# EleutherAI/DALLE-mtf

Measured on AMD Instinct MI355X. Metric: train tokens/sec (text+image) per node, dalle_example, higher is better.
Workload: dtype bf16

## Files before the change

### dalle-mtf_amd/csrc/elementwise.hip

```cpp
#include "common.h"
#include <stdarg.h>

static thread_local char g_err[512] = "ok";
void dmi_set_error(const char* fmt, ...) {
  va_list ap;
  va_start(ap, fmt);
  vsnprintf(g_err, sizeof(g_err), fmt, ap);
  va_end(ap);
}
extern "C" const char* dmi_last_error_string(void) { return g_err; }
extern "C" int dmi_version(void) { return 100; }

__global__ __launch_bounds__(256) void embed_fwd_kernel(const int* __restrict__ tokens,
                                                        const bf16_t* __restrict__ wte,
                                                        const bf16_t* __restrict__ wpe, bf16_t* __restrict__ x,
                                                        int64_t rows, int S, int d, int vocab, const int* __restrict__ pos_dev) {
  const int lane = threadIdx.x & 63, wid = threadIdx.x >> 6;
  const int64_t row = (int64_t)blockIdx.x * 4 + wid;
  if (row >= rows) return;
  int tok = tokens[row];
  tok = tok < 0 ? 0 : (tok >= vocab ? vocab - 1 : tok);
  int s = (int)(row % S);
  if (pos_dev) {
    s = *pos_dev;
    s = s < 0 ? 0 : (s >= S ? S - 1 : s);
  }
  const u32x4* a = (const u32x4*)(wte + (int64_t)tok * d);
  const u32x4* p = (const u32x4*)(wpe + (int64_t)s * d);
  u32x4* o = (u32x4*)(x + row * d);
  for (int c = lane; c < d / 8; c += 64) {
    float fa[8], fp[8];
    unpack8(a[c], fa);
    unpack8(p[c], fp);
#pragma unroll
    for (int j = 0; j < 8; ++j) fa[j] += fp[j];
    o[c] = pack8(fa);
  }
}

extern "C" int dmi_embed_fwd(const int32_t* tokens, const uint16_t* wte, const uint16_t* wpe, uint16_t* x,
                             int64_t rows, int S, int d, int vocab, const int* pos_dev, void* stream) {
  DMI_REQUIRE(tokens && wte && wpe && x, "embed_fwd: null pointer");
  DMI_REQUIRE(d % 8 == 0 && rows > 0 && S > 0, "embed_fwd: d %% 8 != 0 or empty (d=%d rows=%lld)", d, (long long)rows);
  embed_fwd_kernel<<<dim3((unsigned)cdiv64(rows, 4)), dim3(256), 0, (hipStream_t)stream>>>(tokens, wte, wpe, x, rows, S, d, vocab, pos_dev);
  DMI_CHECK_LAUNCH("embed_fwd");
  return DMI_OK;
}

__global__ __launch_bounds__(256) void embed_bwd_wpe_kernel(const bf16_t* __restrict__ dx, float* __restrict__ dwpe,
                                                            int B, int S, int d) {
  const int lane = threadIdx.x & 63, wid = threadIdx.x >> 6;
  const int s = blockIdx.x * 4 + wid;
  if (s >= S) return;
  for (int c = lane; c < d / 8; c += 64) {
    float acc[8] = {0, 0, 0, 0, 0, 0, 0, 0};
    for (int b = 0; b < B; ++b) {
      float f[8];
      unpack8(*(const u32x4*)(dx + ((int64_t)b * S + s) * d + c * 8), f);
#pragma unroll
      for (int j = 0; j < 8; ++j) acc[j] += f[j];
    }
    float* o = dwpe + (int64_t)s * d + c * 8;
    *(f32x4*)o = f32x4{acc[0], acc[1], acc[2], acc[3]};
    *(f32x4*)(o + 4) = f32x4{acc[4], acc[5], acc[6], acc[7]};
  }
}
#define SORT_T 2048
#define SORT_BLK 256
__device__ __forceinline__ int sort_clamp(int k, int vocab) { return k < 0 ? 0 : (k >= vocab ? vocab - 1 : k); }
__global__ __launch_bounds__(SORT_BLK) void sort_count_kernel(const int* __restrict__ keys, int* __restrict__ hist, int n, int vocab,
                                                              int shift, int cpt) {
  __shared__ int col[16][SORT_BLK];
  const int t = threadIdx.x, g = blockIdx.x * SORT_BLK + t;
#pragma unroll
  for (int d = 0; d < 16; ++d) col[d][t] = 0;
  const int i0 = (int64_t)g * cpt < n ? g * cpt : n;
  const int i1 = i0 + cpt < n ? i0 + cpt : n;
  for (int i = i0; i < i1; ++i) col[(sort_clamp(keys[i], vocab) >> shift) & 15][t] += 1;
// ... 1127 lines not shown
      pv[j] -= lr * upd;
    }
    ((f32x4*)p)[i] = pv;
    ((f32x4*)m)[i] = mv;
    ((f32x4*)v)[i] = vv;
    if (pb) *(u32x2*)(pb + i * 4) = u32x2{pack2bf(pv[0], pv[1]), pack2bf(pv[2], pv[3])};
  }
  if (blockIdx.x == 0 && threadIdx.x < (n & 3)) {
    const int64_t i = n4 * 4 + threadIdx.x;
    const float gg = g[i] * mult;
    const float mm = b1 * m[i] + (1.f - b1) * gg;
    const float vv = b2 * v[i] + (1.f - b2) * gg * gg;
    float pp = p[i];
    pp -= lr * (mm / (sqrtf(vv) + eps) + wd * pp);
    p[i] = pp;
    m[i] = mm;
    v[i] = vv;
    if (pb) pb[i] = f2bf(pp);
  }
}
extern "C" int dmi_adam_step(float* p, const float* g, float* m, float* v, uint16_t* p_bf16, int64_t n,
                             const float* gnorm_sq, float clip, float lr, float beta1, float beta2, float eps,
                             float weight_decay, float grad_scale, const float* lr_dev, void* stream) {
  DMI_REQUIRE(p && g && m && v && n > 0, "adam_step: bad args");
  DMI_REQUIRE((((uintptr_t)p | (uintptr_t)g | (uintptr_t)m | (uintptr_t)v) & 15) == 0 && (((uintptr_t)p_bf16) & 7) == 0,
              "adam_step: buffers must be 16-byte aligned");
  int64_t blocks = cdiv64(n / 4 + 1, 256);
  if (blocks > 4096) blocks = 4096;
  adam_kernel<<<dim3((unsigned)blocks), dim3(256), 0, (hipStream_t)stream>>>(p, g, m, v, p_bf16, n, gnorm_sq, clip, lr, beta1, beta2, eps, weight_decay, grad_scale, lr_dev);
  DMI_CHECK_LAUNCH("adam_step");
  return DMI_OK;
}

__global__ __launch_bounds__(256) void cast_kernel(const float* __restrict__ in, bf16_t* __restrict__ out, int64_t n) {
  for (int64_t i = (int64_t)blockIdx.x * 256 + threadIdx.x; i < n; i += (int64_t)gridDim.x * 256) out[i] = f2bf(in[i]);
}
extern "C" int dmi_cast_f32_bf16(const float* in, uint16_t* out, int64_t n, void* stream) {
  DMI_REQUIRE(in && out && n > 0, "cast: bad args");
  int64_t blocks = cdiv64(n, 256);
  if (blocks > 8192) blocks = 8192;
  cast_kernel<<<dim3((unsigned)blocks), dim3(256), 0, (hipStream_t)stream>>>(in, out, n);
  DMI_CHECK_LAUNCH("cast");
  return DMI_OK;
}

__device__ __forceinline__ unsigned order_key(float v) {
  const unsigned u = __float_as_uint(v);
  return (u & 0x80000000u) ? ~u : (u | 0x80000000u);
}
__device__ __forceinline__ float key_value(unsigned k) { return __uint_as_float((k & 0x80000000u) ? (k & 0x7fffffffu) : ~k); }
__device__ __forceinline__ uint64_t splitmix64(uint64_t x) {
  x += 0x9E3779B97F4A7C15ull;
  x = (x ^ (x >> 30)) * 0xBF58476D1CE4E5B9ull;
  x = (x ^ (x >> 27)) * 0x94D049BB133111EBull;
  return x ^ (x >> 31);
}
#define SAMPLE_MAX_VOCAB 8192
__global__ __launch_bounds__(256) void sample_tokens_kernel(const bf16_t* __restrict__ z, int ldz, const bf16_t* __restrict__ bias, int nv,
                                                            float inv_temp, int top_k, uint64_t seed, const unsigned* __restrict__ params_dev,
                                                            int pos_arg, int* pos_dev, int advance, int token_offset,
                                                            int* __restrict__ next_tok, int* __restrict__ out, int out_ld, int out_col0) {
  __shared__ unsigned keys[SAMPLE_MAX_VOCAB];
  __shared__ int cnt[4];
  __shared__ float bval[4];
  __shared__ int bidx[4];
  const int b = blockIdx.x, tid = threadIdx.x, lane = tid & 63, wid = tid >> 6;
// ... 285 lines not shown
```

### dalle-mtf_amd/dalle_hip/__init__.py

```python
from __future__ import annotations

import ctypes
import os
import re
import struct

import numpy as np
from ctypes import c_char_p, c_float, c_int, c_int64, c_void_p

import torch

_HERE = os.path.dirname(os.path.abspath(__file__))
LIB_PATH = os.environ.get("DALLE_HIP_LIB") or os.path.join(_HERE, "libdalle_hip.so")
HEADER_PATH = os.path.join(os.path.dirname(os.path.dirname(_HERE)), "include", "dalle_hip.h")

GEMM_BIAS, GEMM_RELU, GEMM_RESIDUAL, GEMM_RELU_MASK, GEMM_OUT_F32, GEMM_ROWSCALE = 1, 2, 4, 8, 16, 32

_lib = None


class DalleHipError(RuntimeError):
    pass


# ... 31 lines not shown
        "dmi_sort_tokens": (I, [P, P, P, L64, I, P, P]),
        "dmi_embed_bwd_workspace_bytes": (L64, [I, I, I]),
        "dmi_embed_bwd": (I, [P, P, P, P, P, I, I, I, I, P, P]),
        "dmi_layernorm_fwd": (I, [P, P, P, P, P, P, L64, I, F, P]),
        "dmi_layernorm_bwd_workspace_bytes": (L64, [L64, I]),
        "dmi_layernorm_bwd": (I, [P, P, P, P, P, P, P, P, P, P, L64, I, P]),
        "dmi_layernorm_bwd_finish_batch": (I, [P, P, P, P, I, I, P]),
        "dmi_gemm_nt": (I, [P, I, P, I, P, I, I, I, I, I, P, P, P, P, P]),
        "dmi_gemm_nt_splitk_workspace_bytes": (L64, [I, I, I]),
        "dmi_gemm_nt_splitk": (I, [P, I, P, I, P, I, I, I, I, P, P, P]),
        "dmi_gemm_tn_workspace_bytes": (L64, [I, I, I]),
        "dmi_gemm_tn": (I, [P, I, P, I, P, P, P, I, I, I, P, P, P, P]),
        "dmi_gemm_tn_group": (I, [P, I, I, P, P, P]),
        "dmi_gemm_tn_group_plan": (I, [P, P, I, I]),
        "dmi_reduce_slabs_batch": (I, [P, I, P]),
        "dmi_colsum_workspace_bytes": (L64, [L64, I]),
        "dmi_colsum": (I, [P, I, P, L64, I, P, P]),
        "dmi_transpose_bf16": (I, [P, P, I, I, I, P]),
        "dmi_attention_fwd": (I, [P, P, P, I, I, I, P]),
        "dmi_attention_bwd": (I, [P, P, P, P, P, P, I, I, I, P]),
        "dmi_attention_decode": (I, [P, P, P, I, I, I, I, P, P]),
        "dmi_attention_fwd_hd": (I, [P, P, P, I, I, I, I, P]),
        "dmi_attention_bwd_hd": (I, [P, P, P, P, P, P, I, I, I, I, P]),
        "dmi_attention_decode_hd": (I, [P, P, P, I, I, I, I, P, I, P]),
        "dmi_attn_mask_plan": (L64, [P, I, P, L64]),
        "dmi_attention_fwd_masked": (I, [P, P, P, P, P, I, I, I, I, P]),
        "dmi_attention_bwd_masked": (I, [P, P, P, P, P, P, P, P, I, I, I, I, P]),
        "dmi_attention_decode_masked": (I, [P, P, P, P, P, I, I, I, I, P, I, P]),
        "dmi_label_logit": (I, [P, I, P, I, P, P, P, P, L64, I, I, P]),
        "dmi_gemm_nt_softmax_partials": (L64, [I]),
        "dmi_gemm_nt_softmax": (I, [P, I, P, I, P, P, P, I, P, I, I, I, P]),
        "dmi_softmax_finish": (I, [P, I, P, P, P, P, I, P, I, P, P, I, I, P, P, P, P, P, L64, I, I, F, P]),
        "dmi_shift_labels": (I, [P, P, I, I, I, P]),
        "dmi_cross_entropy": (I, [P, I, P, P, P, L64, I, F, P]),
        "dmi_sum_f32": (I, [P, L64, F, P, P]),
        "dmi_assemble_tokens": (I, [P, P, P, I, I, I, I, I, P]),
        "dmi_sample_tokens": (I, [P, I, P, I, I, F, I, ctypes.c_uint64, P, I, P, I, I, P, P, I, I, P]),
        "dmi_sample_tokens_p": (I, [P, I, P, I, I, F, I, ctypes.c_uint64, F, P, I, P, I, I, P, P, I, I, P, P]),
        "dmi_ln_gemm_nt": (I, [P, I, P, P, F, P, I, P, I, I, I, I, I, P, P]),
        "dmi_logits_f32": (I, [P, I, P, P, I, I, P]),
        "dmi_gemm_nt_ln": (I, [P, I, P, I, P, I, I, I, I, P, P, P, P, F, P, I, P, P, P]),
        "dmi_gemm_nt_lnbwd_parts": (I, [I]),
        "dmi_gemm_nt_lnbwd": (I, [P, I, P, I, I, I, I, P, P, P, P, P, P, P, P, I, P, P]),
        "dmi_layernorm_bwd_finish_parts": (I, [P, I, P, P, I, P]),
        "dmi_relu_bits_bytes": (L64, [I, I]),
        "dmi_relu_bits_auto": (I, [I, I, I]),
        "dmi_gemm_nt_ln_auto": (I, [I, I, I]),
        "dmi_gemm_nt_relu_bits": (I, [P, I, P, I, P, I, I, I, I, P, P, P]),
        "dmi_gemm_nt_mask_bits": (I, [P, I, P, I, P, I, I, I, I, P, P]),
        "dmi_sumsq_workspace_bytes": (L64, [L64]),
        "dmi_sumsq": (I, [P, L64, P, P, P]),
        "dmi_adam_step": (I, [P, P, P, P, P, L64, P, F, F, F, F, F, F, F, P, P]),
        "dmi_adafactor_plan": (I, [P, I, P]),
        "dmi_adafactor_step": (I, [P, I, P, P, P, P, P, P, P, F, F, P, F, F, F, F, P, L64, P]),
        "dmi_cast_f32_bf16": (I, [P, P, L64, P]),
        "dmi_transpose_bf16_padded": (I, [P, P, I, I, I, P]),
        "dmi_transpose_bf16_batch": (I, [P, P, P, I, L64, P]),
        "dmi_im2col": (I, [P, P, I, I, I, I, I, I, I, I, P, P, I, P]),
        "dmi_conv_gemm_nt": (I, [P, I, I, I, I, I, I, I, I, P, P, P, I, P, I, I, I, P, P, P, P]),
        "dmi_conv_wgrad_tn_workspace_bytes": (L64, [I, I, I]),
        "dmi_conv_wgrad_tn": (I, [P, I, I, I, I, I, I, I, I, P, P, P, I, I, P, P, P, P, P, P]),
        "dmi_weight_gather": (I, [P, P, I, I, I, P, I, P]),
        "dmi_weight_gather_batch": (I, [P, P, P, I, L64, P]),
        "dmi_pixel_interleave": (I, [P, P, I, I, I, I, P]),
        "dmi_pad_channels": (I, [P, P, L64, I, I, P]),
        "dmi_unpad_channels": (I, [P, P, L64, I, I, P]),
        "dmi_gumbel_softmax_fwd": (I, [P, P, P, P, P, L64, I, F, I, P, P]),
        "dmi_gumbel_softmax_bwd": (I, [P, P, P, L64, I, F, P, P]),
        "dmi_mse_workspace_bytes": (L64, []),
        "dmi_mse_loss": (I, [P, P, P, P, L64, I, I, F, P, P]),
        "dmi_add_f32": (I, [P, P, L64, P]),
        "dmi_comm_load": (I, [c_char_p]),
        "dmi_comm_unique_id_bytes": (I, []),
        "dmi_comm_unique_id": (I, [P]),
        "dmi_comm_init": (I, [P, I, I, P]),
        "dmi_comm_destroy": (I, [P]),
        "dmi_allreduce_bucket": (I, [P, P, L64, P]),
        "dmi_comm_broadcast_f32": (I, [P, P, L64, I, P]),
        "dmi_conv2d_f32": (I, [P, I, I, I, I, I, I, I, I, P, P, P, P, P, P, I, I, P]),
        "dmi_space_to_depth_f32": (I, [P, P, I, I, I, I, I, I, P]),
        "dmi_depth_to_space_f32": (I, [P, P, I, I, I, I, I, I, P]),
        "dmi_crc32c": (ctypes.c_uint32, [c_char_p, ctypes.c_size_t]),
    }
    for name, (res, args) in sig.items():
        fn = getattr(L, name)
# ... 281 lines not shown
        return float(self.host[PLAN_HDR["LIVE_F"]]) / float(self.host[PLAN_HDR["CAUSAL_F"]])

    def live_fraction_dkv(self):
        return float(self.host[PLAN_HDR["LIVE_K"]]) / float(self.host[PLAN_HDR["CAUSAL_K"]])


def attn_mask_plan_bytes(mask_u8, S):
    m = np.ascontiguousarray(mask_u8, dtype=np.uint8)
    return int(lib().dmi_attn_mask_plan(m.ctypes.data, int(S), None, 0))


def attention_fwd_masked(qkv, o, lse, plan, B, H, S, head_dim=128):
    _dev(qkv, o, lse)
    _check(lib().dmi_attention_fwd_masked(_p(qkv), _p(o), _p(lse), _p(plan.dev), plan.host.ctypes.data, B, H, S, int(head_dim),
                                          _stream()), "attention_fwd_masked")


def attention_bwd_masked(qkv, o, d_o, lse, scratch, dqkv, plan, B, H, S, head_dim=128):
    _dev(qkv, o, d_o, lse, scratch, dqkv)
    _check(lib().dmi_attention_bwd_masked(_p(qkv), _p(o), _p(d_o), _p(lse), _p(scratch), _p(dqkv), _p(plan.dev), plan.host.ctypes.data,
                                          B, H, S, int(head_dim), _stream()), "attention_bwd_masked")


def attention_decode_masked(qkv, o, plan, B, H, S, pos, fresh=None, pos_dev=None, head_dim=128):
    _check(lib().dmi_attention_decode_masked(_p(qkv), _p(fresh), _p(o), _p(plan.dev), plan.host.ctypes.data, B, H, S, int(pos),
                                             _p(pos_dev), int(head_dim), _stream()), "attention_decode_masked")


def shift_labels(tokens, labels, B, S, eos):
    _dev(tokens, labels)
    _check(lib().dmi_shift_labels(_p(tokens), _p(labels), B, S, eos, _stream()), "shift_labels")


def cross_entropy(z, ldz, labels, loss_rows, lse, M, V, dz_scale):
    _dev(z, labels, loss_rows)
    _check(lib().dmi_cross_entropy(_p(z), ldz, _p(labels), _p(loss_rows), _p(lse), M, V, dz_scale, _stream()), "cross_entropy")


def label_logit(X, ldx, Wt, ldw, bias, labels, zl, flag, M, K, V):
    _dev(X, Wt, bias, labels, zl, flag)
    _check(lib().dmi_label_logit(_p(X), ldx, _p(Wt), ldw, _p(bias), _p(labels), _p(zl), _p(flag), M, K, V, _stream()), "label_logit")


def gemm_nt_softmax_partials(N):
    return int(lib().dmi_gemm_nt_softmax_partials(N))


def gemm_nt_softmax(X, ldx, Wt, ldw, bias, rowshift, E, lde, rowsum_part, M, N, K):
    _dev(X, Wt, bias, E, rowsum_part)
    _check(lib().dmi_gemm_nt_softmax(_p(X), ldx, _p(Wt), ldw, _p(bias), _p(rowshift), _p(E), lde, _p(rowsum_part), M, N, K,
                                     _stream()), "gemm_nt_softmax")


def softmax_finish(rowsum_part, nparts, label_logit, rowshift, labels, X, ldx, Wt, ldw, bias, E, lde, N, loss_rows, rowscale,
                   rowscale_bf16, Xs, flag, M, K, V, dz_scale):
    _dev(rowsum_part, label_logit, rowshift, labels, X, Wt, bias, E, loss_rows, flag)
    _check(lib().dmi_softmax_finish(_p(rowsum_part), nparts, _p(label_logit), _p(rowshift), _p(labels), _p(X), ldx, _p(Wt), ldw,
                                    _p(bias), _p(E), lde, N,
                                    _p(loss_rows), _p(rowscale), _p(rowscale_bf16), _p(Xs), _p(flag), M, K, V, float(dz_scale),
                                    _stream()), "softmax_finish")


def sum_f32(x, n, scale, out):
    _dev(x, out)
    _check(lib().dmi_sum_f32(_p(x), n, scale, _p(out), _stream()), "sum_f32")

# ... 42 lines not shown
def sample_params(temperature=1.0, top_k=0, seed=0, top_p=None):
    def bits(x):
        return struct.unpack("<I", struct.pack("<f", x))[0]
    words = [bits(1.0 / temperature if temperature > 0 else 0.0), int(top_k), int(seed) & 0xffffffff, (int(seed) >> 32) & 0xffffffff]
    if top_p is not None:
        words += [bits(top_p), 0]
    return torch.tensor([w - (1 << 32) if w >= (1 << 31) else w for w in words], dtype=torch.int32)


def logits_f32(z, ldz, bias, out, B, nv):
    _dev(z, out)
    assert z.dtype == torch.bfloat16 and out.dtype == torch.float32 and out.is_contiguous() and out.numel() >= B * nv
    if bias is not None:
        _dev(bias)
        assert bias.dtype == torch.bfloat16
    _check(lib().dmi_logits_f32(_p(z), int(ldz), _p(bias), _p(out), int(B), int(nv), _stream()), "logits_f32")


def sumsq_workspace_bytes(n):
    return lib().dmi_sumsq_workspace_bytes(n)


def sumsq(g, n, out, ws):
    _dev(g, out, ws)
    _check(lib().dmi_sumsq(_p(g), n, _p(out), _p(ws), _stream()), "sumsq")


def adam_step(p, g, m, v, p_bf16, n, gnorm_sq, clip, lr, beta1, beta2, eps, wd, grad_scale=1.0, lr_dev=None):
    _dev(p, g, m, v)
    _check(lib().dmi_adam_step(_p(p), _p(g), _p(m), _p(v), _p(p_bf16), n, _p(gnorm_sq), clip, lr, beta1, beta2, eps,
                               wd, grad_scale, _p(lr_dev), _stream()), "adam_step")


AF_FIELDS = 17


def adafactor_plan(table):
    assert table.dtype == torch.int64 and not table.is_cuda and table.is_contiguous() and table.shape[1] == AF_FIELDS
    totals = torch.zeros(3, dtype=torch.int64)
    _check(lib().dmi_adafactor_plan(_p(table), table.shape[0], _p(totals)), "adafactor_plan")
    return tuple(int(x) for x in totals)


def adafactor_step(table_dev, nvars, totals, p, g, m, slots, p_bf16, gnorm_sq, clip, lr, decay, beta1, eps1, eps2, ws,
                   lr_dev=None):
    _dev(table_dev, p, g, m, slots, gnorm_sq, ws)
    tot = (ctypes.c_int64 * 3)(*totals)
    _check(lib().dmi_adafactor_step(_p(table_dev), nvars, ctypes.addressof(tot), _p(p), _p(g), _p(m), _p(slots), _p(p_bf16),
                                    _p(gnorm_sq), clip, lr, _p(lr_dev), decay, beta1, eps1, eps2, _p(ws), ws.numel() * ws.element_size(),
                                    _stream()), "adafactor_step")


def cast_f32_bf16(inp, out, n):
    _dev(inp, out)
    _check(lib().dmi_cast_f32_bf16(_p(inp), _p(out), n, _stream()), "cast_f32_bf16")



def transpose_padded(inp, out, R_valid, R_pitch, C):
    _dev(inp, out)
    _check(lib().dmi_transpose_bf16_padded(_p(inp), _p(out), R_valid, R_pitch, C, _stream()), "transpose_padded")


def _iarr(vals):
    return (ctypes.c_int * len(vals))(*[int(v) for v in vals])

# ... 142 lines not shown
```

### dalle-mtf_amd/src/dalle_mtf/engine.py

```python
from __future__ import annotations

import hashlib
import math
import os
from collections import OrderedDict
from typing import Dict, List, Optional, Tuple

import numpy as np
import torch

import dalle_hip as dh
from ..dp import GradReducer

HEAD_DIMS = (64, 128)
ALIGN = 128


def _round_up(x, m):
    return (x + m - 1) // m * m


def adafactor_factored_dims(shape, min_dim_size_to_factor=128):
    if len(shape) < 2:
        return None
# ... 333 lines not shown
                  dh.gemm_tn_workspace_bytes(M, d, d), dh.layernorm_bwd_workspace_bytes(M, d),
                  dh.sumsq_workspace_bytes(self.lay.total), dh.gemm_nt_splitk_workspace_bytes(M // 2 + 256, d, 8))
        self.ws = torch.empty(int(wsz) + 1024, dtype=torch.uint8, device=self.dev)
        self.ws_blk = [torch.empty(int(dh.gemm_tn_workspace_bytes(M, i_, j_)) + 256, dtype=torch.uint8, device=self.dev)
                       for i_, j_ in ((4 * d, d), (d, 4 * d), (d, d), (d, 3 * d))]
        self.deferred = dh.DeferredReduces()
        ln_ok = dh.gemm_nt_ln_auto(M, d, 4 * d) and self.dp_reserve_cus == 0
        self.fuse_ln = bool(self.hp.get("fuse_ln", os.environ.get("DALLE_FUSE_LN", "1") != "0")) and ln_ok
        self.fuse_ln1 = self.fuse_ln and not self.recompute
        self.hp.setdefault("dgrad_tail_split", os.environ.get("DALLE_DGRAD_TAIL", "1") != "0")
        self.hp.setdefault("defer_reduces", os.environ.get("DALLE_DEFER_REDUCES", "1") != "0")
        self.hp.setdefault("wgrad_pair", os.environ.get("DALLE_WGRAD_PAIR", "1") != "0")
        self.hp.setdefault("wgrad_group4", os.environ.get("DALLE_WGRAD_GROUP4", "1") != "0")
        self.wgrad_group4 = bool(self.hp["wgrad_group4"] and self.hp["wgrad_pair"] and self.hp["defer_reduces"]
                                 and dh.gemm_tn_group_plan([(4 * d, d), (d, 4 * d), (d, d), (d, 3 * d)], M) > 0)
        self.hp.setdefault("lnbwd_chain", os.environ.get("DALLE_LNBWD_CHAIN", "1") != "0")
        self.fuse_lnbwd = bool(self.hp.get("fuse_lnbwd", os.environ.get("DALLE_FUSE_LNBWD", "1") != "0")) and ln_ok
        if self.fuse_lnbwd:
            self.lnb_batch = bool(self.hp.get("lnbwd_batch_finish", os.environ.get("DALLE_LNBWD_BATCH", "1") != "0"))
            npart = dh.gemm_nt_lnbwd_parts(M) * 2 * d
            self.lnb_part = [torch.empty(npart, dtype=torch.float32, device=self.dev) for _ in range(2 * L if self.lnb_batch else 1)]
            self.ln_ws_final = torch.empty(int(dh.layernorm_bwd_workspace_bytes(M, d)) + 256, dtype=torch.uint8, device=self.dev)

    def _w(self, name):
        return self.view(self.pb, name)

    def forward(self, tokens: torch.Tensor, need_grad=True) -> torch.Tensor:
        M, d, L, B, H, S, Vp = self.M, self.d, self.L, self.B, self.H, self.S, self.Vp
        assert tokens.shape == (B, S) and tokens.dtype == torch.int32
        self.tokens.copy_(tokens)
        self._sort_done = None
        if need_grad:
            self._launch_sort()
        dh.shift_labels(self.tokens, self.labels, B, S, self.eos)
        dh.embed_fwd(self.tokens, self._w("embedding/wte"), self._w("positional_embedding/wpe"), self.X[0], S, d, self.V)
        for l in range(L):
            self._block_forward(l)
        if not (self.fuse_ln1 and L > 0):
            dh.layernorm_fwd(self.X[L], self._w("to_logits/layer_norm/g"), self._w("to_logits/layer_norm/b"), self.xnf,
                             self.statf[0], self.statf[1], M, d)
        Wt, bias = self.tview("to_logits/linear_out/kernel"), self._w("to_logits/linear_out/bias")
        nmb = (self.hp.get("num_microbatches", 1) or 1) if need_grad else 1
        if need_grad:
            dh.label_logit(self.xnf, d, Wt, d, bias, self.labels, self.zl, self.head_flag, M, d, self.V)
        hook = getattr(self, "event_hook", None)
        if hook is not None:
            e0 = torch.cuda.Event(enable_timing=True)
            e0.record()
        if need_grad:
            dh.gemm_nt_softmax(self.xnf, d, Wt, d, bias, None, self.z, Vp, self.rowsum_part, M, Vp, d)
        else:
            dh.gemm_nt(self.xnf, d, Wt, d, self.z, Vp, M, Vp, d, dh.GEMM_BIAS, bias=bias)
        if hook is not None:
            e1 = torch.cuda.Event(enable_timing=True)
            e1.record()
            hook().append((e0, e1))
        if need_grad:
            dh.softmax_finish(self.rowsum_part, self.nparts, self.zl, None, self.labels, self.xnf, d, Wt, d, bias, self.z, Vp, Vp,
                              self.loss_rows, self.rowscale, self.rowscale_bf, self.xs, self.head_flag, M, d, self.V,
                              1.0 / (self.B_global * S * nmb))
        else:
            dh.cross_entropy(self.z, Vp, self.labels, self.loss_rows, None, M, self.V, 0.0)
        dh.sum_f32(self.loss_rows, M, 1.0 / (M * nmb), self.loss)
        return self.loss

    def _block_forward(self, l):
        M, d, B, H, S, L = self.M, self.d, self.B, self.H, self.S, self.L
        p = f"layer_{l}/"
# ... 405 lines not shown
        self.wait_grads()
        if self.optimizer == "adafactor":
            return self._adafactor_step()
        return self._adam_step()

    def _adafactor_step(self):
        hp = self.hp
        clip = hp.get("gradient_clipping", 1.0)
        lr = self.learning_rate()
        get = lambda k, dflt: dflt if hp.get(k) is None else float(hp[k])
        if self._af_beta1() != 0.0 and self.m is None:
            self.m = torch.zeros(self.lay.total, dtype=torch.float32, device=self.dev)
        dh.adafactor_step(self.af_table, len(self.af_vars), self.af_totals, self.p, self.g, self.m, self.af_slots, self.pb,
                          self.gnorm_sq, 0.0 if clip is None else float(clip), lr, get("weight_decay", 0.0), self._af_beta1(),
                          get("epsilon_1", 1e-30), get("epsilon_2", 1e-3), self.af_ws)
        self.refresh_compute_copies(cast=False)
        self.global_step += 1
        return lr

    def _adam_step(self):
        hp = self.hp
        n = self.lay.total
        clip = hp.get("gradient_clipping", 1.0)
        lr = self.learning_rate()
        b1 = hp.get("beta_1") or 0.9
        b2 = hp.get("beta_2") or 0.999
        eps = hp.get("epsilon") or 1e-6
        wd = hp.get("weight_decay") or 0.0
        gn = None
        cl = 0.0
        if clip is not None:
            dh.sumsq(self.g, n, self.gnorm_sq, self.ws)
            gn, cl = self.gnorm_sq, float(clip)
        if not wd:
            dh.adam_step(self.p, self.g, self.m, self.v, self.pb, n, gn, cl, lr, b1, b2, eps, 0.0)
        else:
            for name, _ in self.lay.entries:
                o, k = self.lay.offset[name], _round_up(self.lay.numel(name), ALIGN)
                use = ("norm" not in name) and ("bias" not in name) and not name.endswith("o_b")
                dh.adam_step(self.p[o:o + k], self.g[o:o + k], self.m[o:o + k], self.v[o:o + k], self.pb[o:o + k], k, gn, cl,
                             lr, b1, b2, eps, wd if use else 0.0)
        self.refresh_compute_copies(cast=False)
        self.global_step += 1
        return lr

    def train_step(self, tokens: torch.Tensor) -> torch.Tensor:
        nmb = self.hp.get("num_microbatches", 1) or 1
        if nmb == 1:
            loss = self.forward(tokens, need_grad=True)
            self.backward()
            self.optimizer_step()
            return loss
        assert tokens.shape == (nmb * self.B, self.S), f"expected {nmb} micro-batches of {self.B} rows"
        if getattr(self, "gacc", None) is None:
            self.gacc = torch.empty_like(self.g)
        if getattr(self, "loss_acc", None) is None:
            self.loss_acc = torch.zeros_like(self.loss)
        self.loss_acc.zero_()
        for i in range(nmb):
            loss = self.forward(tokens[i * self.B:(i + 1) * self.B], need_grad=True)
            self.loss_acc += loss
            self.backward(allreduce=False)
            if i == 0:
                self.gacc.copy_(self.g)
            else:
                dh.add_f32(self.gacc, self.g, self.lay.total)
        self.g.copy_(self.gacc)
        self.reducer.ready(0, self.lay.total)
        self.optimizer_step()
        return self.loss_acc

    def grad_norm(self) -> float:
        return float(torch.sqrt(self.gnorm_sq).item())

    def state_dict(self):
        sd = {"p": self.p.detach().cpu(), "global_step": self.global_step, "optimizer": self.optimizer}
        for k in ("m", "v", "af_slots"):
# ... 18 lines not shown
```

### include/dalle_hip.h

```cpp
#ifndef DALLE_HIP_H
#define DALLE_HIP_H
#include <stddef.h>
#include <stdint.h>
#ifdef __cplusplus
extern "C" {
#endif

typedef enum {
  DMI_OK = 0,
  DMI_ERR_INVALID = -1,
  DMI_ERR_LAUNCH = -2,
  DMI_ERR_UNSUPPORTED = -3
} dmi_status;

const char* dmi_last_error_string(void);
int dmi_version(void);
int dmi_get_option(const char* name);
int dmi_set_option(const char* name, int value);
int dmi_set_debug_buffer(void* device_buffer);

int dmi_embed_fwd(const int32_t* tokens, const uint16_t* wte, const uint16_t* wpe, uint16_t* x,
                  int64_t rows , int S, int d, int vocab, const int* pos_dev, void* stream);
int64_t dmi_sort_tokens_workspace_bytes(int64_t n);
int dmi_sort_tokens(const int32_t* tokens, int32_t* sorted_tokens, int32_t* perm, int64_t n, int vocab,
// ... 32 lines not shown
                int* n_deferred, void* stream);
int dmi_reduce_slabs_batch(const dmi_reduce_item* items, int n, void* stream);
typedef struct dmi_tn_problem { const uint16_t* X; int ldx; const uint16_t* dY; int ldy; float* dW; float* dbias;
                                const uint16_t* bias_weights; int I; int J; void* workspace; } dmi_tn_problem;
int dmi_gemm_tn_group(const dmi_tn_problem* probs, int n, int M, dmi_reduce_item* deferred, int* n_deferred, void* stream);
int dmi_gemm_tn_group_plan(const int* I, const int* J, int n, int M);

int64_t dmi_colsum_workspace_bytes(int64_t M, int N);
int dmi_colsum(const uint16_t* Y, int ldy, float* out, int64_t M, int N, void* workspace, void* stream);
int dmi_transpose_bf16(const uint16_t* in, uint16_t* out, int batch, int R, int C, void* stream);

int dmi_attention_fwd(const uint16_t* qkv, uint16_t* o, float* lse, int B, int H, int S, void* stream);
int dmi_attention_bwd(const uint16_t* qkv, const uint16_t* o, const uint16_t* d_o, const float* lse, float* scratch,
                      uint16_t* dqkv, int B, int H, int S, void* stream);

int dmi_attention_decode(uint16_t* qkv, const uint16_t* fresh, uint16_t* o, int B, int H, int S, int pos, const int* pos_dev,
                         void* stream);
int dmi_attention_fwd_hd(const uint16_t* qkv, uint16_t* o, float* lse, int B, int H, int S, int head_dim, void* stream);
int dmi_attention_bwd_hd(const uint16_t* qkv, const uint16_t* o, const uint16_t* d_o, const float* lse, float* scratch,
                         uint16_t* dqkv, int B, int H, int S, int head_dim, void* stream);
int dmi_attention_decode_hd(uint16_t* qkv, const uint16_t* fresh, uint16_t* o, int B, int H, int S, int pos, const int* pos_dev,
                            int head_dim, void* stream);

int64_t dmi_attn_mask_plan(const uint8_t* mask, int S, int32_t* plan, int64_t plan_bytes);
int dmi_attention_fwd_masked(const uint16_t* qkv, uint16_t* o, float* lse, const int32_t* plan, const int32_t* plan_host, int B, int H,
                             int S, int head_dim, void* stream);
int dmi_attention_bwd_masked(const uint16_t* qkv, const uint16_t* o, const uint16_t* d_o, const float* lse, float* scratch,
                             uint16_t* dqkv, const int32_t* plan, const int32_t* plan_host, int B, int H, int S, int head_dim,
                             void* stream);
int dmi_attention_decode_masked(uint16_t* qkv, const uint16_t* fresh, uint16_t* o, const int32_t* plan, const int32_t* plan_host,
                                int B, int H, int S, int pos, const int* pos_dev, int head_dim, void* stream);

int dmi_shift_labels(const int32_t* tokens, int32_t* labels, int B, int S, int eos, void* stream);
int dmi_cross_entropy(uint16_t* z, int ldz, const int32_t* labels, float* loss_rows, float* lse,
                      int64_t M, int V, float dz_scale, void* stream);
int dmi_label_logit(const uint16_t* X, int ldx, const uint16_t* Wt, int ldw, const uint16_t* bias,
                    const int32_t* labels, float* zl, int32_t* flag, int64_t M, int K, int V, void* stream);
int64_t dmi_gemm_nt_softmax_partials(int N);
int dmi_gemm_nt_ln(const uint16_t* A, int lda, const uint16_t* Bt, int ldb, uint16_t* C, int ldc, int M, int N, int K,
                   const uint16_t* bias, const uint16_t* residual, const uint16_t* gamma, const uint16_t* beta, float eps,
                   uint16_t* Y, int ldy, float* mean, float* rstd, void* stream);
int64_t dmi_relu_bits_bytes(int M, int N);
int dmi_relu_bits_auto(int M, int N, int K);
int dmi_gemm_nt_relu_bits(const uint16_t* A, int lda, const uint16_t* Bt, int ldb, uint16_t* C, int ldc, int M, int N, int K,
                          const uint16_t* bias, void* bits, void* stream);
int dmi_gemm_nt_mask_bits(const uint16_t* A, int lda, const uint16_t* Bt, int ldb, uint16_t* C, int ldc, int M, int N, int K,
                          const void* bits, void* stream);
int dmi_gemm_nt_lnbwd_parts(int M);
int dmi_gemm_nt_ln_auto(int M, int N, int K);
int dmi_gemm_nt_lnbwd(const uint16_t* A, int lda, const uint16_t* Bt, int ldb, int M, int N, int K, const uint16_t* x,
                      const uint16_t* gamma, const float* mean, const float* rstd, const uint16_t* dres, uint16_t* dx,
                      float* part, const uint16_t* B2, int ldb2, uint16_t* C2, void* stream);
int dmi_layernorm_bwd_finish_parts(const float* part, int P, float* dg, float* db, int d, void* stream);
int dmi_gemm_nt_softmax(const uint16_t* X, int ldx, const uint16_t* Wt, int ldw, const uint16_t* bias,
                        const float* rowshift, uint16_t* E, int lde, float* rowsum_part, int M, int N, int K, void* stream);
int dmi_softmax_finish(const float* rowsum_part, int nparts, const float* label_logit, const float* rowshift,
                       const int32_t* labels, const uint16_t* X, int ldx,
                       const uint16_t* Wt, int ldw, const uint16_t* bias, uint16_t* E, int lde, int N,
                       float* loss_rows, float* rowscale, uint16_t* rowscale_bf16, uint16_t* Xs, int32_t* flag,
                       int64_t M, int K, int V, float dz_scale, void* stream);
int dmi_sum_f32(const float* x, int64_t n, float scale, float* out, void* stream);

int dmi_assemble_tokens(const int32_t* text, const float* vae_logits, int32_t* tokens_out,
                        int B, int T, int P, int C, int text_vocab, void* stream);

int dmi_sample_tokens(const uint16_t* z, int ldz, const uint16_t* bias, int B, int nv, float temperature, int top_k,
                      uint64_t seed, const uint32_t* params_dev, int pos, int32_t* pos_dev, int advance, int token_offset,
                      int32_t* next_tok, int32_t* out, int out_ld, int out_col0, void* stream);

int dmi_sample_tokens_p(const uint16_t* z, int ldz, const uint16_t* bias, int B, int nv, float temperature, int top_k,
                        uint64_t seed, float top_p, const uint32_t* params_dev, int pos, int32_t* pos_dev, int advance,
                        int token_offset, int32_t* next_tok, int32_t* out, int out_ld, int out_col0, float* logp, void* stream);

int dmi_logits_f32(const uint16_t* z, int ldz, const uint16_t* bias, float* out, int B, int nv, void* stream);

int64_t dmi_sumsq_workspace_bytes(int64_t n);
int dmi_sumsq(const float* g, int64_t n, float* out, void* workspace, void* stream);
int dmi_adam_step(float* p, const float* g, float* m, float* v, uint16_t* p_bf16, int64_t n,
                  const float* gnorm_sq, float clip, float lr, float beta1, float beta2, float eps,
                  float weight_decay, float grad_scale, const float* lr_dev, void* stream);

#define DMI_AF_FIELDS 17
int dmi_adafactor_plan(int64_t* table, int nvars, int64_t* totals);
int dmi_adafactor_step(const int64_t* table_dev, int nvars, const int64_t* totals, float* p, const float* g, float* m,
                       float* slots, uint16_t* p_bf16, float* gnorm_sq, float clip, float lr, const float* lr_dev,
                       float decay, float beta1, float eps1, float eps2, void* workspace, int64_t workspace_bytes, void* stream);

int dmi_comm_load(const char* librccl_path);
int dmi_comm_unique_id_bytes(void);
int dmi_comm_unique_id(void* id_out);
int dmi_comm_init(void** comm_out, int nranks, int rank, const void* unique_id);
int dmi_comm_destroy(void* comm);
int dmi_allreduce_bucket(void* comm, float* g, int64_t n, void* stream);
int dmi_comm_broadcast_f32(void* comm, float* buf, int64_t n, int root, void* stream);

int dmi_cast_f32_bf16(const float* in, uint16_t* out, int64_t n, void* stream);

int dmi_transpose_bf16_batch(const uint16_t* in_base, uint16_t* out_base, const int64_t* table, int n,
                             int64_t total_tiles, void* stream);

int dmi_transpose_bf16_padded(const uint16_t* in, uint16_t* out, int R_valid, int R_pitch, int C, void* stream);

int dmi_conv_gemm_nt(const uint16_t* x, int B, int H, int W, int C, int Ho, int Wo, int stride, int ntaps,
                     const int* dy, const int* dx, const uint16_t* Wt, int ldw, uint16_t* out, int ldc, int N,
                     int flags, const uint16_t* bias, const uint16_t* residual, const uint16_t* relu_src, void* stream);

int64_t dmi_conv_wgrad_tn_workspace_bytes(int M, int K, int N);
int dmi_conv_wgrad_tn(const uint16_t* x, int B, int H, int W, int C, int Ho, int Wo, int stride, int ntaps,
                      const int* dy, const int* dx, const uint16_t* dY, int ldy, int N, float* dW, float* dbias,
                      void* workspace, dmi_reduce_item* deferred, int* n_deferred, void* stream);

int dmi_im2col(const uint16_t* x, uint16_t* out, int B, int H, int W, int C, int Ho, int Wo, int stride,
               int ntaps, const int* dy, const int* dx, int ldo, void* stream);
// ... 28 lines not shown
```

Before: 2.876 million.

## Fuse Adam step with transposed bf16 weight copy and fold label shift into embedding

Adds a tiled Adam kernel that updates fp32 master weights and writes both the bf16 copy and the transposed bf16 copy through a shared-memory tile. This replaces the separate refresh_compute_copies transpose pass. It also computes shifted labels inside the embedding forward kernel, removing one launch. The tile layout needs a per-parameter plan table and a binary search for every block.

```diff
diff --git a/dalle-mtf_amd/csrc/elementwise.hip b/dalle-mtf_amd/csrc/elementwise.hip
--- a/dalle-mtf_amd/csrc/elementwise.hip
+++ b/dalle-mtf_amd/csrc/elementwise.hip
@@ -14,13 +14,15 @@
 __global__ __launch_bounds__(256) void embed_fwd_kernel(const int* __restrict__ tokens,
                                                         const bf16_t* __restrict__ wte,
                                                         const bf16_t* __restrict__ wpe, bf16_t* __restrict__ x,
-                                                        int64_t rows, int S, int d, int vocab, const int* __restrict__ pos_dev) {
+                                                        int64_t rows, int S, int d, int vocab, const int* __restrict__ pos_dev,
+                                                        int* __restrict__ labels, int eos) {
   const int lane = threadIdx.x & 63, wid = threadIdx.x >> 6;
   const int64_t row = (int64_t)blockIdx.x * 4 + wid;
   if (row >= rows) return;
   int tok = tokens[row];
   tok = tok < 0 ? 0 : (tok >= vocab ? vocab - 1 : tok);
   int s = (int)(row % S);
+  if (labels && lane == 0) labels[row] = (s == S - 1) ? eos : tokens[row + 1];
   if (pos_dev) {
     s = *pos_dev;
     s = s < 0 ? 0 : (s >= S ? S - 1 : s);
@@ -42,8 +44,19 @@
                              int64_t rows, int S, int d, int vocab, const int* pos_dev, void* stream) {
   DMI_REQUIRE(tokens && wte && wpe && x, "embed_fwd: null pointer");
   DMI_REQUIRE(d % 8 == 0 && rows > 0 && S > 0, "embed_fwd: d %% 8 != 0 or empty (d=%d rows=%lld)", d, (long long)rows);
-  embed_fwd_kernel<<<dim3((unsigned)cdiv64(rows, 4)), dim3(256), 0, (hipStream_t)stream>>>(tokens, wte, wpe, x, rows, S, d, vocab, pos_dev);
+  embed_fwd_kernel<<<dim3((unsigned)cdiv64(rows, 4)), dim3(256), 0, (hipStream_t)stream>>>(tokens, wte, wpe, x, rows, S, d, vocab, pos_dev,
+                                                                                             nullptr, 0);
   DMI_CHECK_LAUNCH("embed_fwd");
+  return DMI_OK;
+}
+extern "C" int dmi_embed_fwd_labels(const int32_t* tokens, const uint16_t* wte, const uint16_t* wpe, uint16_t* x, int32_t* labels,
+                                    int64_t rows, int S, int d, int vocab, int eos, void* stream) {
+  DMI_REQUIRE(tokens && wte && wpe && x && labels, "embed_fwd_labels: null pointer");
+  DMI_REQUIRE(d % 8 == 0 && rows > 0 && S > 0 && rows % S == 0, "embed_fwd_labels: d %% 8 != 0, empty or rows %% S != 0 (d=%d rows=%lld S=%d)",
+              d, (long long)rows, S);
+  embed_fwd_kernel<<<dim3((unsigned)cdiv64(rows, 4)), dim3(256), 0, (hipStream_t)stream>>>(tokens, wte, wpe, x, rows, S, d, vocab, nullptr,
+                                                                                             labels, eos);
+  DMI_CHECK_LAUNCH("embed_fwd_labels");
   return DMI_OK;
 }
 
@@ -1237,6 +1250,142 @@
   return DMI_OK;
 }
 
+#define ADAM_FB 4096
+__device__ __forceinline__ float adam_mult(const float* __restrict__ gnorm_sq, float clip, float gscale) {
+  float mult = gscale;
+  if (gnorm_sq != nullptr && clip > 0.f) {
+    const float gn = sqrtf(gnorm_sq[0]) * gscale;
+    mult = gscale * (clip / fmaxf(gn, clip));
+  }
+  return mult;
+}
+__device__ __forceinline__ void adam4(float* __restrict__ p, const float* __restrict__ g, float* __restrict__ m,
+                                      float* __restrict__ v, float mult, float lr, float b1, float b2, float eps, float wd,
+                                      f32x4& pv) {
+  pv = *(f32x4*)p;
+  const f32x4 gv = *(const f32x4*)g;
+  f32x4 mv = *(f32x4*)m, vv = *(f32x4*)v;
+#pragma unroll
+  for (int j = 0; j < 4; ++j) {
+    const float gg = gv[j] * mult;
+    mv[j] = fmaf(b1, mv[j], (1.f - b1) * gg);
+    vv[j] = fmaf(b2, vv[j], ((1.f - b2) * gg) * gg);
+    float upd = mv[j] / (sqrtf(vv[j]) + eps);
+    upd = fmaf(wd, pv[j], upd);
+    pv[j] = fmaf(-lr, upd, pv[j]);
+  }
+  *(f32x4*)p = pv;
+  *(f32x4*)m = mv;
+  *(f32x4*)v = vv;
+}
+__global__ __launch_bounds__(256) void adam_t_kernel(float* __restrict__ p, const float* __restrict__ g,
+                                                     float* __restrict__ m, float* __restrict__ v,
+                                                     bf16_t* __restrict__ pb, bf16_t* __restrict__ pbt,
+                                                     const int64_t* __restrict__ table, int n,
+                                                     const float* __restrict__ gnorm_sq, float clip, float lr, float b1,
+                                                     float b2, float eps, float wd, float gscale,
+                                                     const float* __restrict__ lr_dev) {
+  __shared__ unsigned t[64][33];
+  if (lr_dev) lr = lr_dev[0];
+  const float mult = adam_mult(gnorm_sq, clip, gscale);
+  const int64_t blk = blockIdx.x;
+  int lo = 0, hi = n - 1;
+  while (lo < hi) {
+    const int mid = (lo + hi + 1) >> 1;
+    if (table[mid * 5 + 4] <= blk) lo = mid; else hi = mid - 1;
+  }
+  const int64_t off = table[lo * 5], t_off = table[lo * 5 + 1], R = table[lo * 5 + 2], C = table[lo * 5 + 3];
+  const int64_t local = blk - table[lo * 5 + 4];
+  const int tid = threadIdx.x;
+  if (t_off < 0) {
+    const int64_t b0 = off + local * ADAM_FB, end = min(off + R, b0 + ADAM_FB);
+    for (int64_t e = b0 + tid * 4; e < end; e += 1024) {
+      f32x4 pv;
+      adam4(p + e, g + e, m + e, v + e, mult, lr, b1, b2, eps, wd, pv);
+      *(u32x2*)(pb + e) = u32x2{pack2bf(pv[0], pv[1]), pack2bf(pv[2], pv[3])};
+    }
+    return;
+  }
+  const int64_t tc = (C + 63) / 64;
+  const int r0 = (int)(local / tc) * 64, c0 = (int)(local % tc) * 64;
+  const int cq = (tid & 15) * 4, rq = tid >> 4;
+  unsigned short* th = (unsigned short*)&t[0][0];
+#pragma unroll
+  for (int q = 0; q < 4; ++q) {
+    const int r = rq + 16 * q;
+    if (r0 + r < R && c0 + cq < C) {
+      const int64_t e = off + (int64_t)(r0 + r) * C + c0 + cq;
+      f32x4 pv;
+      adam4(p + e, g + e, m + e, v + e, mult, lr, b1, b2, eps, wd, pv);
+      const unsigned w01 = pack2bf(pv[0], pv[1]), w23 = pack2bf(pv[2], pv[3]);
+      *(u32x2*)(pb + e) = u32x2{w01, w23};
+      th[(cq + 0) * 66 + r] = (unsigned short)(w01 & 0xffffu);
+      th[(cq + 1) * 66 + r] = (unsigned short)(w01 >> 16);
+      th[(cq + 2) * 66 + r] = (unsigned short)(w23 & 0xffffu);
+      th[(cq + 3) * 66 + r] = (unsigned short)(w23 >> 16);
+    }
+  }
+  __syncthreads();
+  const int orow = tid >> 2, seg = tid & 3;
+  const int c = c0 + orow, r = r0 + 16 * seg;
+  if (c < C) {
+#pragma unroll
+    for (int q = 0; q < 2; ++q) {
+      const int rr = r + 8 * q;
+      if (rr < R) {
+        u32x4 w;
+#pragma unroll
+        for (int i = 0; i < 4; ++i) w[i] = t[orow][8 * seg + 4 * q + i];
+        *(u32x4*)(pbt + t_off + (int64_t)c * R + rr) = w;
+      }
+    }
+  }
+}
+
+extern "C" int dmi_adam_t_plan(int64_t* table, int n, int64_t total, int64_t t_total, int64_t* blocks_out) {
+  DMI_REQUIRE(table && blocks_out && n > 0 && total > 0 && t_total >= 0, "adam_t_plan: bad args");
+  int64_t at = 0, blocks = 0;
+  for (int i = 0; i < n; ++i) {
+    int64_t* e = table + (int64_t)i * 5;
+    const int64_t off = e[0], t_off = e[1], R = e[2], C = e[3];
+    DMI_REQUIRE(off == at, "adam_t_plan: entry %d starts at %lld, the previous one ends at %lld", i, (long long)off, (long long)at);
+    DMI_REQUIRE(off % 4 == 0 && R > 0, "adam_t_plan: entry %d: offset not a multiple of 4 or empty", i);
+    if (t_off < 0) {
+      DMI_REQUIRE(t_off == -1 && R % 4 == 0, "adam_t_plan: plain entry %d: t_off must be -1, length a multiple of 4", i);
+      e[4] = blocks;
+      blocks += cdiv64(R, ADAM_FB);
+      at += R;
+    } else {
+      DMI_REQUIRE(C > 0 && C % 4 == 0 && R % 8 == 0 && t_off % 8 == 0,
+                  "adam_t_plan: matrix entry %d: C %% 4, R %% 8 and t_off %% 8 must be 0 (R=%lld C=%lld)", i, (long long)R, (long long)C);
+      DMI_REQUIRE(t_off + R * C <= t_total, "adam_t_plan: matrix entry %d: [out,in] copy past the end of its buffer", i);
+      e[4] = blocks;
+      blocks += cdiv64(R, 64) * cdiv64(C, 64);
+      at += R * C;
+    }
+  }
+  DMI_REQUIRE(at == total, "adam_t_plan: the entries cover %lld of %lld elements", (long long)at, (long long)total);
+  DMI_REQUIRE(blocks < ((int64_t)1 << 31), "adam_t_plan: too many blocks");
+  *blocks_out = blocks;
+  return DMI_OK;
+}
+
+extern "C" int dmi_adam_step_t(float* p, const float* g, float* m, float* v, uint16_t* p_bf16, uint16_t* p_bf16_t,
+                               const int64_t* table_dev, int n, int64_t blocks, const float* gnorm_sq, float clip, float lr,
+                               float beta1, float beta2, float eps, float weight_decay, float grad_scale, const float* lr_dev,
+                               void* stream) {
+  DMI_REQUIRE(p && g && m && v && p_bf16 && p_bf16_t && table_dev && n > 0 && blocks > 0 && blocks < ((int64_t)1 << 31),
+              "adam_step_t: bad args");
+  DMI_REQUIRE((((uintptr_t)p | (uintptr_t)g | (uintptr_t)m | (uintptr_t)v | (uintptr_t)p_bf16_t) & 15) == 0 &&
+                  (((uintptr_t)p_bf16) & 7) == 0,
+              "adam_step_t: buffers must be 16-byte aligned");
+  adam_t_kernel<<<dim3((unsigned)blocks), dim3(256), 0, (hipStream_t)stream>>>(
+      p, g, m, v, (bf16_t*)p_bf16, (bf16_t*)p_bf16_t, table_dev, n, gnorm_sq, clip, lr, beta1, beta2, eps, weight_decay, grad_scale,
+      lr_dev);
+  DMI_CHECK_LAUNCH("adam_step_t");
+  return DMI_OK;
+}
+
 __global__ __launch_bounds__(256) void cast_kernel(const float* __restrict__ in, bf16_t* __restrict__ out, int64_t n) {
   for (int64_t i = (int64_t)blockIdx.x * 256 + threadIdx.x; i < n; i += (int64_t)gridDim.x * 256) out[i] = f2bf(in[i]);
 }
diff --git a/dalle-mtf_amd/dalle_hip/__init__.py b/dalle-mtf_amd/dalle_hip/__init__.py
--- a/dalle-mtf_amd/dalle_hip/__init__.py
+++ b/dalle-mtf_amd/dalle_hip/__init__.py
@@ -87,6 +87,7 @@
         "dmi_gemm_nt_softmax": (I, [P, I, P, I, P, P, P, I, P, I, I, I, P]),
         "dmi_softmax_finish": (I, [P, I, P, P, P, P, I, P, I, P, P, I, I, P, P, P, P, P, L64, I, I, F, P]),
         "dmi_shift_labels": (I, [P, P, I, I, I, P]),
+        "dmi_embed_fwd_labels": (I, [P, P, P, P, P, L64, I, I, I, I, P]),
         "dmi_cross_entropy": (I, [P, I, P, P, P, L64, I, F, P]),
         "dmi_sum_f32": (I, [P, L64, F, P, P]),
         "dmi_assemble_tokens": (I, [P, P, P, I, I, I, I, I, P]),
@@ -106,6 +107,8 @@
         "dmi_sumsq_workspace_bytes": (L64, [L64]),
         "dmi_sumsq": (I, [P, L64, P, P, P]),
         "dmi_adam_step": (I, [P, P, P, P, P, L64, P, F, F, F, F, F, F, F, P, P]),
+        "dmi_adam_t_plan": (I, [P, I, L64, L64, P]),
+        "dmi_adam_step_t": (I, [P, P, P, P, P, P, P, I, L64, P, F, F, F, F, F, F, F, P, P]),
         "dmi_adafactor_plan": (I, [P, I, P]),
         "dmi_adafactor_step": (I, [P, I, P, P, P, P, P, P, P, F, F, P, F, F, F, F, P, L64, P]),
         "dmi_cast_f32_bf16": (I, [P, P, L64, P]),
@@ -453,6 +456,12 @@
     _check(lib().dmi_shift_labels(_p(tokens), _p(labels), B, S, eos, _stream()), "shift_labels")
 
 
+def embed_fwd_labels(tokens, wte, wpe, x, labels, S, d, vocab, eos):
+    _dev(tokens, wte, wpe, x, labels)
+    _check(lib().dmi_embed_fwd_labels(_p(tokens), _p(wte), _p(wpe), _p(x), _p(labels), tokens.numel(), S, d, vocab, eos, _stream()),
+           "embed_fwd_labels")
+
+
 def cross_entropy(z, ldz, labels, loss_rows, lse, M, V, dz_scale):
     _dev(z, labels, loss_rows)
     _check(lib().dmi_cross_entropy(_p(z), ldz, _p(labels), _p(loss_rows), _p(lse), M, V, dz_scale, _stream()), "cross_entropy")
@@ -561,6 +570,20 @@
                                wd, grad_scale, _p(lr_dev), _stream()), "adam_step")
 
 
+def adam_t_plan(table, total, t_total):
+    assert table.dtype == torch.int64 and not table.is_cuda and table.is_contiguous() and table.shape[1] == 5
+    blocks = ctypes.c_int64(0)
+    _check(lib().dmi_adam_t_plan(_p(table), table.shape[0], total, t_total, ctypes.addressof(blocks)), "adam_t_plan")
+    return int(blocks.value)
+
+
+def adam_step_t(p, g, m, v, p_bf16, p_bf16_t, table_dev, blocks, gnorm_sq, clip, lr, beta1, beta2, eps, wd, grad_scale=1.0,
+                lr_dev=None):
+    _dev(p, g, m, v, p_bf16, p_bf16_t, table_dev)
+    _check(lib().dmi_adam_step_t(_p(p), _p(g), _p(m), _p(v), _p(p_bf16), _p(p_bf16_t), _p(table_dev), table_dev.shape[0], blocks,
+                                 _p(gnorm_sq), clip, lr, beta1, beta2, eps, wd, grad_scale, _p(lr_dev), _stream()), "adam_step_t")
+
+
 AF_FIELDS = 17
 
 
diff --git a/dalle-mtf_amd/src/dalle_mtf/engine.py b/dalle-mtf_amd/src/dalle_mtf/engine.py
--- a/dalle-mtf_amd/src/dalle_mtf/engine.py
+++ b/dalle-mtf_amd/src/dalle_mtf/engine.py
@@ -389,8 +389,8 @@
         self._sort_done = None
         if need_grad:
             self._launch_sort()
-        dh.shift_labels(self.tokens, self.labels, B, S, self.eos)
-        dh.embed_fwd(self.tokens, self._w("embedding/wte"), self._w("positional_embedding/wpe"), self.X[0], S, d, self.V)
+        dh.embed_fwd_labels(self.tokens, self._w("embedding/wte"), self._w("positional_embedding/wpe"), self.X[0], self.labels, S, d,
+                            self.V, self.eos)
         for l in range(L):
             self._block_forward(l)
         if not (self.fuse_ln1 and L > 0):
@@ -862,6 +862,13 @@
         if clip is not None:
             dh.sumsq(self.g, n, self.gnorm_sq, self.ws)
             gn, cl = self.gnorm_sq, float(clip)
+        if not wd and self.hp.get("adam_t", os.environ.get("DALLE_ADAM_T", "1") != "0"):
+            if getattr(self, "_adam_t", None) is None:
+                self._adam_t = self._adam_t_table()
+            table, blocks = self._adam_t
+            dh.adam_step_t(self.p, self.g, self.m, self.v, self.pb, self.pbt, table, blocks, gn, cl, lr, b1, b2, eps, 0.0)
+            self.global_step += 1
+            return lr
         if not wd:
             dh.adam_step(self.p, self.g, self.m, self.v, self.pb, n, gn, cl, lr, b1, b2, eps, 0.0)
         else:
@@ -873,6 +880,27 @@
         self.refresh_compute_copies(cast=False)
         self.global_step += 1
         return lr
+
+    def _adam_t_table(self):
+        rows = []
+
+        def plain(o, k):
+            if rows and rows[-1][1] < 0 and rows[-1][0] + rows[-1][2] == o:
+                rows[-1][2] += k
+            elif k > 0:
+                rows.append([o, -1, k, 0, 0])
+        for name, _ in self.lay.entries:
+            o, k = self.lay.offset[name], self.lay.numel(name)
+            kp = _round_up(k, ALIGN)
+            if name in self.lay.t_offset:
+                r, c = self.lay.shape[name]
+                rows.append([o, self.lay.t_offset[name], r, c, 0])
+                plain(o + k, kp - k)
+            else:
+                plain(o, kp)
+        table = torch.tensor(rows, dtype=torch.int64)
+        blocks = dh.adam_t_plan(table, self.lay.total, self.lay.t_total)
+        return table.to(self.dev), blocks
 
     def train_step(self, tokens: torch.Tensor) -> torch.Tensor:
         nmb = self.hp.get("num_microbatches", 1) or 1
diff --git a/include/dalle_hip.h b/include/dalle_hip.h
--- a/include/dalle_hip.h
+++ b/include/dalle_hip.h
@@ -88,6 +88,8 @@
                                 int B, int H, int S, int pos, const int* pos_dev, int head_dim, void* stream);
 
 int dmi_shift_labels(const int32_t* tokens, int32_t* labels, int B, int S, int eos, void* stream);
+int dmi_embed_fwd_labels(const int32_t* tokens, const uint16_t* wte, const uint16_t* wpe, uint16_t* x, int32_t* labels,
+                         int64_t rows, int S, int d, int vocab, int eos, void* stream);
 int dmi_cross_entropy(uint16_t* z, int ldz, const int32_t* labels, float* loss_rows, float* lse,
                       int64_t M, int V, float dz_scale, void* stream);
 int dmi_label_logit(const uint16_t* X, int ldx, const uint16_t* Wt, int ldw, const uint16_t* bias,
@@ -135,6 +137,10 @@
 int dmi_adam_step(float* p, const float* g, float* m, float* v, uint16_t* p_bf16, int64_t n,
                   const float* gnorm_sq, float clip, float lr, float beta1, float beta2, float eps,
                   float weight_decay, float grad_scale, const float* lr_dev, void* stream);
+int dmi_adam_t_plan(int64_t* table, int n, int64_t total, int64_t t_total, int64_t* blocks_out);
+int dmi_adam_step_t(float* p, const float* g, float* m, float* v, uint16_t* p_bf16, uint16_t* p_bf16_t,
+                    const int64_t* table_dev, int n, int64_t blocks, const float* gnorm_sq, float clip, float lr,
+                    float beta1, float beta2, float eps, float weight_decay, float grad_scale, const float* lr_dev, void* stream);
 
 #define DMI_AF_FIELDS 17
 int dmi_adafactor_plan(int64_t* table, int nvars, int64_t* totals);
```

New measurement: 2.892 million (median of 6 runs). No clear change (+0.6%).
